# hackmad/pbrt-v3-rs

Measured on AMD Instinct MI355X. Metric: Mrays/s, higher is better.
Workload: dtype f32

## Files before the change

include/pbrt_hip.h:

```cpp
#ifndef PBRT_HIP_H
#define PBRT_HIP_H

#include <stddef.h>
#include <stdint.h>

#ifdef __cplusplus
extern "C" {
#endif

typedef struct PbrtHipScene PbrtHipScene;

enum {
    PBRT_HIP_OK = 0,
    PBRT_HIP_ERR_INVALID_ARG = -1,
    PBRT_HIP_ERR_STATE = -2,
    PBRT_HIP_ERR_DEVICE = -3,
    PBRT_HIP_ERR_NO_DEVICE = -4,
    PBRT_HIP_ERR_UNSUPPORTED = -5,
    PBRT_HIP_ERR_OOM = -6
};

typedef struct PbrtHipRay {
    float o[3];
    float t_max;
// ... 146 lines not shown
int pbrt_hip_occluded_batch_device(PbrtHipScene*, const void* d_rays, void* d_occluded, uint64_t n, float* kernel_ms);

int pbrt_hip_set_traversal_counting(PbrtHipScene*, int on);
int pbrt_hip_get_traversal_counts(PbrtHipScene*, uint64_t out[8]);

int pbrt_hip_render_path(PbrtHipScene*, int max_depth, float rr_threshold, int light_strategy,
                         const int pixel_bounds[4], int tile_size, int tile_part, int tile_parts,
                         float* out_xyz, float* out_weight, PbrtHipStats* out_stats);

int pbrt_hip_render_whitted(PbrtHipScene*, int max_depth, const int pixel_bounds[4], int tile_size, int tile_part, int tile_parts,
                            float* out_xyz, float* out_weight, PbrtHipStats* out_stats);

int pbrt_hip_set_sample_record_budget(PbrtHipScene*, uint64_t bytes);
int pbrt_hip_get_render_footprint(PbrtHipScene*, uint64_t out[8]);

int pbrt_hip_tile_buffer_floats(PbrtHipScene*, int tile_size, int tile_part, int tile_parts, uint64_t* out_floats);
int pbrt_hip_render_path_tiles_device(PbrtHipScene*, int max_depth, float rr_threshold, int light_strategy,
                                      const int pixel_bounds[4], int tile_size, int tile_part, int tile_parts,
                                      void* d_tile_buffer, PbrtHipStats* out_stats);
int pbrt_hip_merge_tiles_device(PbrtHipScene*, int tile_size, int tile_parts, const void* const* d_tile_buffers,
                                float* out_xyz, float* out_weight);

int pbrt_hip_film_to_rgb(const PbrtHipScene*, const float* xyz, const float* weight, float* out_rgb);

int pbrt_hip_generate_camera_rays(PbrtHipScene*, const int pixel_bounds[4], uint32_t sample_index,
                                  PbrtHipRay* out_rays, float* out_pfilm_xy);

int pbrt_hip_bsdf_probe_batch(PbrtHipScene*, uint32_t material, int op, int path, uint64_t n, const float* wo , const float* wi , const float* u ,
                              const uint32_t* flags , const float* frame , float* out );
int pbrt_hip_sampler_value_batch(PbrtHipScene*, uint64_t n, const int* xy , const uint32_t* sample , const uint32_t* dim , int use_lds, float* out );
#define PBRT_HIP_LIGHT_PROBE_STRIDE 28
int pbrt_hip_light_probe_batch(PbrtHipScene*, uint32_t light, int op, int variant, uint64_t n, const float* ref , const float* u , const float* wi ,
                               float* out );

#ifdef __cplusplus
}
#endif
#endif
```

pbrt-v3-rs_amd/csrc/probe.hip:

```cpp
#define PH_OUTLINE_MATH 1
#include "scene_host.h"
#include "pt_device.h"
#include "bsdf_general.h"
#include "wf_device.h"
#include "texture.h"
#include "sphere_light.h"
#include <cstring>

namespace ph {

struct ProbeFrame { float ns[3], ng[3], ss[3]; };
#define PH_PROBE_BLOCK 128

template <bool GEN>
__global__ __launch_bounds__(PH_PROBE_BLOCK) void bsdf_probe_kernel(DeviceScene sc, uint32_t material, int op, uint32_t n, const float* wo_in, const float* wi_in, const float* u_in,
                                                                   const uint32_t* flags_in, ProbeFrame fr, float* out) {
    const uint32_t i = blockIdx.x * blockDim.x + threadIdx.x;
    if (i >= n) return;
    SurfHit si;
    si.p = mk3(0.0f, 0.0f, 0.0f); si.p_error = si.p; si.wo = si.p; si.time = 0.0f; si.prim = 0u;
    si.ns = ld3(fr.ns); si.n = ld3(fr.ng); si.dpdu_s = ld3(fr.ss);
    const f3 wo = ld3(wo_in + 3 * (size_t)i), wi = ld3(wi_in + 3 * (size_t)i);
    const f2 u = mk2(u_in[2 * (size_t)i], u_in[2 * (size_t)i + 1]);
    const uint32_t flags = flags_in[i];
// ... 178 lines not shown
    const LightRec& l = s->lights[light];
    if (l.type == PH_L_AREA) {
        if (l.prim >= s->tri_mesh.size()) return set_err(s, PBRT_HIP_ERR_STATE, "light_probe_batch: the area light has no shape yet");
        if ((s->meshes[s->tri_mesh[l.prim]].flags & PH_MESH_QUADRIC) && variant != 2)
            return set_err(s, PBRT_HIP_ERR_UNSUPPORTED, "light_probe_batch: a spherical area light is sampled by the Whitted light loop alone (variant 2)");
    }
    if (variant == 1 && l.map_mip1) return set_err(s, PBRT_HIP_ERR_UNSUPPORTED, "light_probe_batch: variant 1 is the code of scenes without textures; this light holds a radiance, projection or goniometric map");
    if (n == 0) return PBRT_HIP_OK;
    PH_CHECK(s, hipSetDevice(s->device));
    int rc;
    if ((rc = upload_scene(s))) return rc;
    const size_t stride = PBRT_HIP_LIGHT_PROBE_STRIDE * sizeof(float);
    const size_t o_ref = 0, o_u = o_ref + up256(n * 40), o_wi = o_u + up256(n * 8), o_out = o_wi + up256(n * 12), total = o_out + up256(n * stride);
    Scratch sx;
    PH_CHECK(s, hipMalloc(&sx.p, total));
    char* d = static_cast<char*>(sx.p);
    PH_CHECK(s, hipMemcpyAsync(d + o_ref, ref, n * 40, hipMemcpyHostToDevice, s->stream));
    PH_CHECK(s, hipMemcpyAsync(d + o_u, u, n * 8, hipMemcpyHostToDevice, s->stream));
    PH_CHECK(s, hipMemcpyAsync(d + o_wi, wi, n * 12, hipMemcpyHostToDevice, s->stream));
    const dim3 grid((uint32_t)((n + PH_PROBE_BLOCK - 1) / PH_PROBE_BLOCK)), block(PH_PROBE_BLOCK);
    auto launch = [&](auto kernel) {
        hipLaunchKernelGGL(kernel, grid, block, 0, s->stream, s->ds, light, op, (uint32_t)n, (const float*)(d + o_ref), (const float*)(d + o_u), (const float*)(d + o_wi), (float*)(d + o_out));
    };
    if (variant == 0) launch(ph::light_probe_kernel<0>);
    else if (variant == 1) launch(ph::light_probe_kernel<1>);
    else launch(ph::light_probe_kernel<2>);
    PH_CHECK(s, hipGetLastError());
    PH_CHECK(s, hipMemcpyAsync(out, d + o_out, n * stride, hipMemcpyDeviceToHost, s->stream));
    PH_CHECK(s, hipStreamSynchronize(s->stream));
    return PBRT_HIP_OK;
    });
}

}
```

pbrt-v3-rs_amd/csrc/raysort.h:

```cpp
#pragma once
#include "traverse.h"

namespace ph {

#define PH_SORT_BINS 4096u
#define PH_SORT_KEYS (2u * PH_SORT_BINS)
#define PH_SORT_BLOCK 256

struct RaySortParams {
    const uint32_t* keys_cl; const uint32_t* keys_sh;
    const uint32_t* n_cl; const uint32_t* n_sh;
    uint32_t* order;
    uint32_t* bin_start;
    uint32_t* bin_cursor;
};
struct RaySortGrid {
    float lo[3], scale[3];
};

PH_DEV uint32_t part1by2(uint32_t v) {
    v &= 0xFu;
    v = (v | (v << 4)) & 0xC3u;
    v = (v | (v << 2)) & 0x249u;
    return v;
}

PH_DEV uint32_t ray_sort_key(const RaySortGrid& g, float ox, float oy, float oz) {
    const float fx = (ox - g.lo[0]) * g.scale[0], fy = (oy - g.lo[1]) * g.scale[1], fz = (oz - g.lo[2]) * g.scale[2];
    const uint32_t cx = (uint32_t)pmini(pmaxi((int)(fx * 16.0f), 0), 15);
    const uint32_t cy = (uint32_t)pmini(pmaxi((int)(fy * 16.0f), 0), 15);
    const uint32_t cz = (uint32_t)pmini(pmaxi((int)(fz * 16.0f), 0), 15);
    return part1by2(cx) | (part1by2(cy) << 1) | (part1by2(cz) << 2);
}
PH_DEV uint32_t raysort_key_at(const RaySortParams& p, uint32_t i, uint32_t n_cl) {
    return i < n_cl ? p.keys_cl[i] : PH_SORT_BINS + p.keys_sh[i - n_cl];
}

PH_DEV void raysort_slice(const RaySortParams& p, uint32_t n, uint32_t& lo, uint32_t& hi) {
    const uint32_t per = (((n + gridDim.x - 1u) / gridDim.x) + PH_SORT_BLOCK - 1u) & ~(uint32_t)(PH_SORT_BLOCK - 1u);
    lo = blockIdx.x * per; hi = lo + per < n ? lo + per : n;
    if (lo > n) lo = n;
}

__global__ __launch_bounds__(PH_SORT_BLOCK) void raysort_hist_kernel(RaySortParams p) {
    __shared__ uint32_t h[PH_SORT_KEYS];
    const uint32_t n_cl = *p.n_cl, n = n_cl + *p.n_sh;
    uint32_t lo, hi;
    raysort_slice(p, n, lo, hi);
    if (lo >= hi) return;
    for (uint32_t k = threadIdx.x; k < PH_SORT_KEYS; k += PH_SORT_BLOCK) h[k] = 0u;
    __syncthreads();
    for (uint32_t i = lo + threadIdx.x; i < hi; i += PH_SORT_BLOCK) atomicAdd(&h[raysort_key_at(p, i, n_cl)], 1u);
    __syncthreads();
    for (uint32_t k = threadIdx.x; k < PH_SORT_KEYS; k += PH_SORT_BLOCK)
        if (h[k]) atomicAdd(&p.bin_start[k], h[k]);
}

__global__ __launch_bounds__(1024) void raysort_scan_kernel(RaySortParams p) {
    __shared__ uint32_t part[1024];
    constexpr uint32_t PER = PH_SORT_KEYS / 1024u;
    uint32_t v[PER], sum = 0u;
    for (uint32_t k = 0; k < PER; k++) { v[k] = p.bin_start[threadIdx.x * PER + k]; sum += v[k]; }
    part[threadIdx.x] = sum;
    __syncthreads();
    for (uint32_t o = 1; o < 1024u; o <<= 1) {
        const uint32_t add = threadIdx.x >= o ? part[threadIdx.x - o] : 0u;
        __syncthreads();
        part[threadIdx.x] += add;
        __syncthreads();
    }
    uint32_t run = part[threadIdx.x] - sum;
    for (uint32_t k = 0; k < PER; k++) { p.bin_start[threadIdx.x * PER + k] = run; p.bin_cursor[threadIdx.x * PER + k] = 0u; run += v[k]; }
}

__global__ __launch_bounds__(PH_SORT_BLOCK) void raysort_scatter_kernel(RaySortParams p) {
    __shared__ uint32_t h[PH_SORT_KEYS];
    __shared__ uint32_t base[PH_SORT_KEYS];
    const uint32_t n_cl = *p.n_cl, n = n_cl + *p.n_sh;
    uint32_t lo, hi;
    raysort_slice(p, n, lo, hi);
    if (lo >= hi) return;
    for (uint32_t k = threadIdx.x; k < PH_SORT_KEYS; k += PH_SORT_BLOCK) h[k] = 0u;
    __syncthreads();
    for (uint32_t i = lo + threadIdx.x; i < hi; i += PH_SORT_BLOCK) atomicAdd(&h[raysort_key_at(p, i, n_cl)], 1u);
    __syncthreads();
    for (uint32_t k = threadIdx.x; k < PH_SORT_KEYS; k += PH_SORT_BLOCK) {
        const uint32_t c = h[k];
        base[k] = c ? p.bin_start[k] + atomicAdd(&p.bin_cursor[k], c) : 0u;
        h[k] = 0u;
    }
    __syncthreads();
    for (uint32_t i = lo + threadIdx.x; i < hi; i += PH_SORT_BLOCK) {
        const uint32_t key = raysort_key_at(p, i, n_cl);
        p.order[base[key] + atomicAdd(&h[key], 1u)] = i;
    }
}

}
```

pbrt-v3-rs_amd/csrc/scene_host.h:

```cpp
#pragma once
#include "../../include/pbrt_hip.h"
#include "band_plan.h"
#include "bvh_build.h"
#include "guard.h"
#include "scene_types.h"
#include <hip/hip_runtime.h>
namespace ph { struct TravParams; }
#include <string>
#include <vector>

struct DevBuf {
    void* p = nullptr;
    size_t bytes = 0;
};

struct SceneHostState {
    std::vector<float> P, N, S, UV;
    bool any_n = false, any_s = false, any_uv = false;
    std::vector<uint32_t> idx, tri_mesh, tri_flags;
    std::vector<MeshRec> meshes;
    std::vector<QuadricRec> quadrics;
    std::vector<float> quadric_bounds;
    std::vector<uint32_t> prim_quadric;
    std::vector<MaterialRec> materials;
    std::vector<LobeRec> lobes;
    struct TextureHost { std::vector<TexOp> prog; int stack_need = 1; };
    std::vector<TextureHost> textures;
    std::vector<MipRec> mipmaps;
    std::vector<Texel> texels;
    struct MaterialParams { int lobe[4] = {-1, -1, -1, -1}; int field[4] = {0, 0, 0, 0}; int lobe2[4] = {-1, -1, -1, -1}; int field2[4] = {0, 0, 0, 0}; bool has_pre = false; float pre[3] = {1, 1, 1}; int rough_lobe = -1, rough_lobe2 = -1; bool rough_remap = false;
                            int made_as = 0;   float raw_k[4][3] = {{0, 0, 0}, {0, 0, 0}, {0, 0, 0}, {0, 0, 0}}; float raw_eta = 1.5f, raw_ur = 0, raw_vr = 0;
                            bool raw_remap = false, rebuilt = false; int mix_n1 = 0; };
    std::vector<MaterialParams> material_params;
    bool alpha_textures = false;
    bool alpha_lean = false;
    bool bump_materials = false;
    bool textured_materials = false;
// ... 33 lines not shown
    MultiDevice* multi = nullptr;

    DeviceScene ds{};
    std::vector<void*> owned;
    void* tree_dev_nodes = nullptr; void* tree_dev_tris = nullptr; size_t tree_dev_n_tris = 0;
    bool uploaded = false;
    int light_strategy_uploaded = -1;
    DevBuf d_ld_func, d_ld_cdf;

    DevBuf d_counter, d_spill, d_error, d_rays_tmp, d_out_tmp;
    uint32_t trav_blocks = 0;
    bool count_traversal = false;
    DevBuf d_counts;
    hipEvent_t ev0 = nullptr, ev1 = nullptr;

    struct Wavefront* wf = nullptr;
    struct WhittedWorkspace* wh = nullptr;

    uint64_t record_budget = 0;
    uint64_t footprint[8] = {0, 0, 0, 0, 0, 0, 0, 0};
};

namespace phost {
int set_err(PbrtHipScene* s, int code, const std::string& msg);
int hip_fail(PbrtHipScene* s, hipError_t e, const char* what);
int ensure_buf(PbrtHipScene* s, DevBuf& b, size_t bytes);
int upload_scene(PbrtHipScene* s);
void projection_light_setup(float fov_deg, float aspect, float out_proj[16], float out_screen[4], float* out_cos_total_width);
void hmip_lookup_triangle(const PbrtHipScene* s, const MipRec& m, float u, float v, float width, float out[3]);
int upload_light_distribution(PbrtHipScene* s, int light_strategy);
int launch_traverse(PbrtHipScene* s, bool anyhit, const void* d_rays, void* d_out, uint32_t n, float* kernel_ms);
void launch_traverse_kernel(PbrtHipScene* s, int mode, uint32_t blocks, const ph::TravParams& p);
int ensure_traversal_workspace(PbrtHipScene* s);
void free_wavefront(PbrtHipScene* s);
int build_hlbvh_device(const BuildInput& in, int max_prims_in_node, hipStream_t stream, BuildOutput& out, std::string& err, const ForestSpec* forest = nullptr,
                       std::vector<ForestTreeOut>* trees_out = nullptr);
int build_sah_device(const BuildInput& in, int max_prims_in_node, hipStream_t stream, BuildOutput& out, std::string& err, void** keep_nodes = nullptr, void** keep_tris = nullptr,
                     const ForestSpec* forest = nullptr, std::vector<ForestTreeOut>* trees_out = nullptr);
void free_tree_dev(PbrtHipScene* s);
int uber_rebuild_for_opacity(PbrtHipScene* s, uint32_t material);
int glass_rebuild_for_roughness(PbrtHipScene* s, uint32_t material);
int translucent_rebuild_rt(PbrtHipScene* s, uint32_t material);
#define PH_MAX_TILE_PARTS 64
int check_render_args(PbrtHipScene* s, int max_depth, int light_strategy, const int* pixel_bounds, int tile_size, int part, int parts);
size_t tile_buffer_floats_for(const PbrtHipScene* s, int tile_size, int part, int parts);
int render_tiles(PbrtHipScene* s, int max_depth, float rr_threshold, int light_strategy, const int pixel_bounds[4], int tile_size, int part, int parts, void* d_tile_buffer,
                 PbrtHipStats* out_stats);
int merge_tiles(PbrtHipScene* s, int tile_size, int parts, const void* const* d_bufs, float* out_xyz, float* out_weight);
DevBuf& tile_buffer_of(PbrtHipScene* s);
int merge_own_tiles(PbrtHipScene* s, int tile_size, int tile_part, int tile_parts, float* out_xyz, float* out_weight);
struct SampleRecords { uint32_t n_px; const int2* px_xy; float4* rec_L; float* rec_py; uint8_t* px_rounded; SampleBand band; uint32_t band_px; std::vector<SampleBand> bands; };
int samples_begin(PbrtHipScene* s, int tile_size, int part, int parts, SampleRecords* out);
int samples_plan_bands(PbrtHipScene* s, SampleRecords* out, size_t chunk_held, size_t chunk_per_path);
int samples_alloc(PbrtHipScene* s, SampleRecords* out);
int samples_band(PbrtHipScene* s, const SampleRecords& r, size_t band, SampleRecords* out);
int samples_to_tiles(PbrtHipScene* s, const SampleRecords& r, void* d_tile_buffer);
size_t path_chunk_bytes_per_path(bool general_materials, bool textured_materials);
void free_whitted(PbrtHipScene* s);
size_t whitted_chunk_bytes_per_sample(uint32_t n_frames);
int spatial_voxels_touched(PbrtHipScene* s, std::vector<uint8_t>& touched, uint64_t* count);
int render_path_multi(PbrtHipScene* s, int max_depth, float rr_threshold, int light_strategy, const int pixel_bounds[4], int tile_size, int tile_part, int tile_parts,
                      float* out_xyz, float* out_weight, PbrtHipStats* out_stats);
void free_multi(PbrtHipScene* s);
}

#define PH_CHECK(s, call)                                              \
// ... 5 lines not shown
```

pbrt-v3-rs_amd/csrc/wavefront.hip:

```cpp
#define PH_OUTLINE_MATH 1
#include "host_math.h"
#include "pt_device.h"
#include "scene_host.h"
#include "spatial.h"
#include "bsdf_general.h"
#include "texture.h"
#include "raysort.h"
#include "phase_clock.h"
#include "matsort.h"
#include "wf_device.h"
#include "chunk_plan.h"
#include <algorithm>
#include <cstdlib>

namespace ph {

enum : uint32_t { F_EXT = 1u, F_PSH = 2u, F_PMIS = 4u, F_SPEC = 8u, F_NODIFF = 16u };

struct IterCounters {
    uint32_t n_cl, n_sh, n_live, head_cl, head_sh, pad[3];
};
struct DevStats { unsigned long long camera_rays, paths_total, paths_zero; };

struct TileInfo {
// ... 666 lines not shown
    int tiles_key[12] = {0}; bool tiles_valid = false;
    DevBuf d_tiles, d_px, d_rays_cl[2], d_hits, d_rays_sh, d_occ, d_live[2], d_ctr, d_stats, d_cam, d_tex_out;
    DevBuf d_sL, d_sbeta, d_sA, d_sf2, d_sbold, d_sidx, d_sprev, d_recL, d_recpy, d_rounded, d_tilebuf, d_xyz, d_w;
    DevBuf d_vox_slot, d_sp_pool, d_sp_list, d_sp_ctr, d_sp_halton;
    DevBuf d_order, d_sort_bins, d_heads, d_keys_cl, d_keys_sh;
    DevBuf d_morder, d_mkeys, d_mbins;
    size_t n_vox = 0;
    std::vector<hipEvent_t> events;
    phost::ChunkTable chunk_table(bool textured, bool mat_queues) {
        const size_t ray = sizeof(ph::RayIn), hit = sizeof(ph::HitOut);
        return {{&d_rays_cl[0], 2 * ray}, {&d_rays_cl[1], 2 * ray}, {&d_hits, 2 * hit}, {&d_rays_sh, ray}, {&d_occ, 1}, {&d_live[0], 4}, {&d_live[1], 4},
                {&d_sL, 2 * 16}, {&d_sbeta, 2 * 16}, {&d_sA, 2 * 16}, {&d_sf2, 2 * 16}, {&d_sbold, 2 * 16}, {&d_sidx, 2 * 16}, {&d_sprev, 2 * 4},
                {&d_order, 3 * 4}, {&d_keys_cl, 2 * 4}, {&d_keys_sh, 4}, {&d_tex_out, textured ? sizeof(TexOut) : 0, textured}, {&d_morder, 4, mat_queues}, {&d_mkeys, 2, mat_queues}};
    }
    std::vector<DevBuf*> all_bufs() {
        std::vector<DevBuf*> v{&d_tiles, &d_px, &d_ctr, &d_stats, &d_cam, &d_recL, &d_recpy, &d_rounded, &d_tilebuf, &d_xyz, &d_w,
                               &d_vox_slot, &d_sp_pool, &d_sp_list, &d_sp_ctr, &d_sp_halton, &d_sort_bins, &d_heads, &d_mbins};
        for (const phost::ChunkBuf& c : chunk_table(false, false)) v.push_back(c.buf);
        return v;
    }
};

namespace phost {

void free_wavefront(PbrtHipScene* s) {
    Wavefront* w = s->wf;
    if (!w) return;
    for (DevBuf* b : w->all_bufs()) release_buf(*b);
    for (hipEvent_t e : w->events) (void)hipEventDestroy(e);
    delete w;
    s->wf = nullptr;
}

size_t path_chunk_bytes_per_path(bool general, bool textured) { Wavefront w; return chunk_bytes_per_path(w.chunk_table(textured, general || textured)); }
static int sat_i(float v) { if (v != v) return 0; if (v >= 2147483648.0f) return 2147483647; if (v <= -2147483648.0f) return (int)0x80000000; return (int)v; }

struct TileGrid { int sb[4]; int ntx, nty; uint32_t slot_w, slot_h; };
static TileGrid tile_grid(const FilmRec& f, int tile_size) {
    TileGrid g;
    g.sb[0] = sat_i(std::floor((float)f.crop[0] + 0.5f - f.radius[0])); g.sb[1] = sat_i(std::floor((float)f.crop[1] + 0.5f - f.radius[1]));
    g.sb[2] = sat_i(std::ceil((float)f.crop[2] - 0.5f + f.radius[0])); g.sb[3] = sat_i(std::ceil((float)f.crop[3] - 0.5f + f.radius[1]));
    g.ntx = std::max((g.sb[2] - g.sb[0] + tile_size - 1) / tile_size, 0); g.nty = std::max((g.sb[3] - g.sb[1] + tile_size - 1) / tile_size, 0);
    const int e_lo_x = sat_i(std::floor(0.5f + f.radius[0])), e_hi_x = sat_i(std::floor(f.radius[0] - 0.5f)) + 1;
    const int e_lo_y = sat_i(std::floor(0.5f + f.radius[1])), e_hi_y = sat_i(std::floor(f.radius[1] - 0.5f)) + 1;
    g.slot_w = (uint32_t)std::max(tile_size + e_lo_x + e_hi_x, 1); g.slot_h = (uint32_t)std::max(tile_size + e_lo_y + e_hi_y, 1);
    return g;
}

static int setup_tiles(PbrtHipScene* s, int tile_size, int part, int parts) {
    if (!s->wf) s->wf = new Wavefront();
    Wavefront& w = *s->wf;
    const FilmRec& f = s->film;
    const TileGrid g = tile_grid(f, tile_size);
    int key[12] = {f.crop[0], f.crop[1], f.crop[2], f.crop[3], 0, 0, tile_size, part, parts, g.ntx, g.nty, 1};
    std::memcpy(&key[4], &f.radius[0], 4); std::memcpy(&key[5], &f.radius[1], 4);
    if (w.tiles_valid && std::memcmp(key, w.tiles_key, sizeof key) == 0) return PBRT_HIP_OK;
    w.tiles_valid = false;
    const int* sb = g.sb; const int ntx = g.ntx, nty = g.nty;
    w.tiles.clear(); w.px_xy.clear();
    std::memcpy(w.sb, sb, sizeof(w.sb)); w.ntx = ntx; w.nty = nty; w.tile_size = tile_size; w.part = part; w.parts = parts;
    w.slot_w = g.slot_w; w.slot_h = g.slot_h;
    for (int t = part; t < ntx * nty; t += parts) {
        ph::TileInfo ti{};
        const int tx = t % ntx, ty = t / ntx;
        ti.tb[0] = sb[0] + tx * tile_size; ti.tb[2] = std::min(ti.tb[0] + tile_size, sb[2]);
        ti.tb[1] = sb[1] + ty * tile_size; ti.tb[3] = std::min(ti.tb[1] + tile_size, sb[3]);
// ... 95 lines not shown
                        int parts, void* d_tile_buffer, PbrtHipStats* out_stats) {
    int rc;
    PH_CHECK(s, hipSetDevice(s->device));
    if ((rc = upload_scene(s))) return rc;
    const bool spatial = light_strategy == 2 && s->lights.size() > 1;
    if ((rc = upload_light_distribution(s, light_strategy == 2 ? 0 : light_strategy))) return rc;
    if (out_stats) std::memset(out_stats, 0, sizeof(*out_stats));
    SampleRecords rec{};
    if ((rc = samples_begin(s, tile_size, part, parts, &rec))) return rc;
    Wavefront& w = *s->wf;
    const uint32_t spp = s->sampler.spp;
    if (rec.n_px == 0) { PH_CHECK(s, hipMemsetAsync(d_tile_buffer, 0, tile_buffer_floats_for(s, tile_size, part, parts) * 4, s->stream)); PH_CHECK(s, hipStreamSynchronize(s->stream)); return PBRT_HIP_OK; }

    static const ChunkPolicy kChunks{128u << 20, 1u << 20, 0x7FFF0000ull, "render"};
    const bool mat_queues = s->general_materials || s->textured_materials;
    const ChunkTable chunk = w.chunk_table(s->textured_materials, mat_queues);
    if ((rc = samples_plan_bands(s, &rec, chunk_bytes_held(chunk), chunk_bytes_per_path(chunk)))) return rc;
    const uint32_t n_px = rec.band_px;
    const size_t rec_need = (size_t)n_px * spp * 20, rec_have = w.d_recL.bytes + w.d_recpy.bytes;
    uint32_t chunk_spp = plan_chunk_spp_now(kChunks, chunk, rec_need > rec_have ? rec_need - rec_have : 0, n_px, spp);
    const int n_iter = max_depth + 1;
    const int kMaxNullSkips = 1024;
    const int n_iter_cap = s->has_none_material ? n_iter + kMaxNullSkips : n_iter;
    const bool has_quadrics = !s->quadrics.empty();
    if ((rc = ensure_buf(s, w.d_ctr, (size_t)(n_iter_cap + 2) * sizeof(ph::IterCounters)))) return rc;
    if ((rc = ensure_buf(s, w.d_stats, 64 + 6 * PHC_N * 8))) return rc;
    if ((rc = samples_alloc(s, &rec))) return rc;
    if ((rc = chunk_alloc_or_halve(s, kChunks, chunk, n_px, chunk_spp))) return rc;
    const size_t B = (size_t)n_px * chunk_spp;
    chunk_note_footprint(s, B, chunk);

    if ((rc = ensure_traversal_workspace(s))) return rc;
    const uint32_t n_heads = 8, head_chunk = 49152, sort_blocks = 1024;
    ph::RaySortParams sortp{};
    ph::RaySortGrid sort_grid{};
    if ((rc = ensure_buf(s, w.d_sort_bins, 2 * PH_SORT_KEYS * 4))) return rc;
    sortp.order = (uint32_t*)w.d_order.p; sortp.bin_start = (uint32_t*)w.d_sort_bins.p; sortp.bin_cursor = sortp.bin_start + PH_SORT_KEYS;
    sortp.keys_cl = (const uint32_t*)w.d_keys_cl.p; sortp.keys_sh = (const uint32_t*)w.d_keys_sh.p;
    for (int k = 0; k < 3; k++) {
        const float ext = s->bvh.root_hi[k] - s->bvh.root_lo[k];
        sort_grid.lo[k] = s->bvh.root_lo[k]; sort_grid.scale[k] = ext > 0.0f ? 1.0f / ext : 0.0f;
    }
    if ((rc = ensure_buf(s, w.d_heads, (size_t)(n_iter_cap + 2) * n_heads * 64))) return rc;
    ph::MatSortParams msp{};
    if (mat_queues) {
        if ((rc = ensure_buf(s, w.d_mbins, (size_t)(2 * PH_MS_BINS + 1) * 4))) return rc;
        msp.max_depth = max_depth; msp.mat_key = s->ds.mat_key; msp.key_emit = s->ds.ms_key_emit; msp.key_idle = s->ds.ms_key_idle;
        msp.tris = s->ds.tris; msp.meshes = s->ds.meshes; msp.hits = (const ph::HitOut*)w.d_hits.p;
        msp.keys = (uint16_t*)w.d_mkeys.p; msp.order = (uint32_t*)w.d_morder.p;
        msp.bin_start = (uint32_t*)w.d_mbins.p; msp.bin_cursor = msp.bin_start + PH_MS_BINS + 1;
    }

    ph::WfParams wp{};
    wp.cam = s->cam; wp.sp = s->sampler;
    wp.textured = s->textured_materials ? 1u : 0u; wp.cam_dev = nullptr;
    wp.any_rt = 0u;
    for (const MaterialRec& mr : s->materials) if (mr.rt_mode) wp.any_rt = 1u;
    if (s->textured_materials) {
        if ((rc = ensure_buf(s, w.d_cam, sizeof(CameraRec)))) return rc;
        PH_CHECK(s, hipMemcpyAsync(w.d_cam.p, &s->cam, sizeof(CameraRec), hipMemcpyHostToDevice, s->stream));
        wp.cam_dev = (const CameraRec*)w.d_cam.p;
    }
    for (int i = 0; i < 4; i++) wp.pixel_bounds[i] = pixel_bounds[i];
    wp.max_depth = max_depth; wp.rr_threshold = rr_threshold;
    wp.rays_cl[0] = (ph::RayIn*)w.d_rays_cl[0].p; wp.rays_cl[1] = (ph::RayIn*)w.d_rays_cl[1].p;
    wp.hits_cl = (ph::HitOut*)w.d_hits.p; wp.rays_sh = (ph::RayIn*)w.d_rays_sh.p; wp.occ = (uint8_t*)w.d_occ.p;
    wp.live[0] = (uint32_t*)w.d_live[0].p; wp.live[1] = (uint32_t*)w.d_live[1].p;
    wp.ctr = (ph::IterCounters*)w.d_ctr.p; wp.stats = (ph::DevStats*)w.d_stats.p;
    for (int k = 0; k < 2; k++) {
        wp.s_L[k] = (float4*)w.d_sL.p + (size_t)k * B; wp.s_beta[k] = (float4*)w.d_sbeta.p + (size_t)k * B; wp.s_A[k] = (float4*)w.d_sA.p + (size_t)k * B;
        wp.s_f2[k] = (float4*)w.d_sf2.p + (size_t)k * B; wp.s_bold[k] = (float4*)w.d_sbold.p + (size_t)k * B; wp.s_idx[k] = (uint4*)w.d_sidx.p + (size_t)k * B;
// ... 27 lines not shown
    uint64_t regular = 0, shadow = 0;
    std::vector<ph::IterCounters> hctr((size_t)n_iter_cap + 2);
    const uint32_t shade_blocks = (uint32_t)std::min<size_t>((B + 255) / 256, 256 * 16);
    wp.tex_out = nullptr;
    if (s->textured_materials) wp.tex_out = (TexOut*)w.d_tex_out.p;

    for (size_t band = 0; band < rec.bands.size(); band++) {
        SampleRecords br{};
        if ((rc = samples_band(s, rec, band, &br))) return rc;
        wp.n_px = br.n_px; wp.px_xy = br.px_xy; wp.rec_L = br.rec_L; wp.rec_py = br.rec_py; wp.px_rounded = br.px_rounded;
        for (uint32_t s0 = 0; s0 < spp; s0 += chunk_spp) {
            const uint32_t cs = std::min(chunk_spp, spp - s0);
            wp.chunk_spp = cs; wp.s0 = s0; wp.B = br.n_px * cs; wp.identity_slots = identity ? 1u : 0u;
            PH_CHECK(s, hipMemsetAsync(w.d_ctr.p, 0, (size_t)(n_iter_cap + 2) * sizeof(ph::IterCounters), s->stream));
            PH_CHECK(s, hipMemsetAsync(w.d_heads.p, 0, (size_t)(n_iter_cap + 2) * n_heads * 64, s->stream));
            if (identity) hipLaunchKernelGGL(ph::preset_counters_kernel, dim3(1), dim3(1), 0, s->stream, wp.ctr, wp.stats, wp.B);
            if ((rc = timed(2, [&]() { hipLaunchKernelGGL(ph::raygen_kernel, dim3((wp.B + 255) / 256), dim3(256), 0, s->stream, s->ds, wp); }))) return rc;
            int iters_run = 0;
            for (int it = 0; it < n_iter_cap; it++) {
                ph::IterCounters* c = (ph::IterCounters*)w.d_ctr.p + it;
                if (it >= n_iter) {
                    uint32_t live = 0;
                    PH_CHECK(s, hipMemcpyAsync(&live, &c->n_live, 4, hipMemcpyDeviceToHost, s->stream));
                    PH_CHECK(s, hipStreamSynchronize(s->stream));
                    if (live == 0) break;
                    if (it == n_iter_cap - 1) return set_err(s, PBRT_HIP_ERR_UNSUPPORTED, "render: a path crossed more than 1024 'none' surfaces");
                }
                iters_run = it + 1;
                ph::TravParams tp{};
                tp.rays = wp.rays_cl[it & 1]; tp.out = wp.hits_cl; tp.n = 0; tp.n_ptr = &c->n_cl; tp.counter = &c->head_cl;
                tp.heads = (uint32_t*)w.d_heads.p + (size_t)it * n_heads * 16; tp.n_heads = n_heads; tp.head_chunk = head_chunk;
                if (it > 0) {
                    tp.rays2 = wp.rays_sh; tp.out2 = wp.occ; tp.n2_ptr = &c->n_sh;
                    sortp.n_cl = &c->n_cl; sortp.n_sh = &c->n_sh;
                    if ((rc = timed(3, [&]() {
                            (void)hipMemsetAsync(sortp.bin_start, 0, PH_SORT_KEYS * 4, s->stream);
                            hipLaunchKernelGGL(ph::raysort_hist_kernel, dim3(sort_blocks), dim3(PH_SORT_BLOCK), 0, s->stream, sortp);
                            hipLaunchKernelGGL(ph::raysort_scan_kernel, dim3(1), dim3(1024), 0, s->stream, sortp);
                            hipLaunchKernelGGL(ph::raysort_scatter_kernel, dim3(sort_blocks), dim3(PH_SORT_BLOCK), 0, s->stream, sortp);
                        }))) return rc;
                    tp.order = sortp.order;
                    if ((rc = timed(0, [&]() { launch_traverse_kernel(s, 2, s->trav_blocks, tp); }))) return rc;
                } else if ((rc = timed(0, [&]() { launch_traverse_kernel(s, 0, s->trav_blocks, tp); }))) return rc;
                if (mat_queues) {
                    msp.s_idx = wp.s_idx[it & 1]; msp.n_live = &c->n_live;
                    if ((rc = timed(2, [&]() {
                            (void)hipMemsetAsync(msp.bin_start, 0, (PH_MS_BINS + 1) * 4, s->stream);
                            hipLaunchKernelGGL(ph::matsort_hist_kernel, dim3(sort_blocks), dim3(PH_MS_BLOCK), 0, s->stream, msp);
                            hipLaunchKernelGGL(ph::matsort_scan_kernel, dim3(1), dim3(PH_MS_BINS), 0, s->stream, msp);
                            hipLaunchKernelGGL(ph::matsort_scatter_kernel, dim3(sort_blocks), dim3(PH_MS_BLOCK), 0, s->stream, msp);
                        }))) return rc;
                }
                if (s->textured_materials) {
                    if ((rc = timed(2, [&]() {
                            const dim3 g(shade_blocks), b(PH_TEX_LDS_THREADS);
                            if (it == 0) {
                                if (has_quadrics) hipLaunchKernelGGL((ph::texture_kernel<false, true, 2, true>), g, b, 0, s->stream, s->ds, wp, it);
                                else if (s->simple_textures) hipLaunchKernelGGL((ph::texture_kernel<true, true, 3>), g, b, 0, s->stream, s->ds, wp, it);
                                else hipLaunchKernelGGL((ph::texture_kernel<false, true, 2>), g, b, 0, s->stream, s->ds, wp, it);
                            } else {
                                if (has_quadrics) hipLaunchKernelGGL((ph::texture_kernel<false, false, 3, true>), g, b, 0, s->stream, s->ds, wp, it);
                                else if (s->simple_textures) hipLaunchKernelGGL((ph::texture_kernel<true, false, 4>), g, b, 0, s->stream, s->ds, wp, it);
                                else hipLaunchKernelGGL((ph::texture_kernel<false, false, 3>), g, b, 0, s->stream, s->ds, wp, it);
                            }
                        }))) return rc;
                }
                if (spatial && (it < max_depth || s->has_none_material)) {
                    if ((rc = timed(2, [&]() {
                            if (has_quadrics) hipLaunchKernelGGL(ph::spatial_mark_kernel<true>, dim3(shade_blocks), dim3(256), 0, s->stream, s->ds, wp, it);
                            else hipLaunchKernelGGL(ph::spatial_mark_kernel<false>, dim3(shade_blocks), dim3(256), 0, s->stream, s->ds, wp, it);
                            hipLaunchKernelGGL(ph::spatial_compute_kernel, dim3(1024), dim3(PH_SPATIAL_BLOCK), 0, s->stream, s->ds, wp.spatial);
                        }))) return rc;
                }
                if ((rc = timed(2, [&]() {
// ... 281 lines not shown
```

pbrt-v3-rs_amd/pbrt_hip/__init__.py:

```python
from __future__ import annotations

import ctypes as C
import os
from dataclasses import dataclass

import numpy as np

_HERE = os.path.dirname(os.path.abspath(__file__))
LIB_PATH = os.environ.get("PBRT_HIP_LIB") or os.path.join(os.path.dirname(_HERE), "libpbrt_hip.so")

OK = 0
ERR_INVALID_ARG, ERR_STATE, ERR_DEVICE, ERR_NO_DEVICE, ERR_UNSUPPORTED, ERR_OOM = -1, -2, -3, -4, -5, -6

RAY_DTYPE = np.dtype([("o", "<f4", 3), ("t_max", "<f4"), ("d", "<f4", 3), ("time", "<f4")])
HIT_DTYPE = np.dtype([("t", "<f4"), ("prim", "<u4"), ("b0", "<f4"), ("b1", "<f4"), ("b2", "<f4"), ("pad", "<u4", 3)])
assert RAY_DTYPE.itemsize == 32 and HIT_DTYPE.itemsize == 32


class Stats(C.Structure):
    _fields_ = [
        ("camera_rays", C.c_uint64), ("regular_rays", C.c_uint64), ("shadow_rays", C.c_uint64),
        ("paths_zero_radiance", C.c_uint64), ("paths_total", C.c_uint64),
        ("render_seconds", C.c_double), ("extend_seconds", C.c_double), ("shadow_seconds", C.c_double),
        ("shade_seconds", C.c_double), ("extend_launches", C.c_uint64), ("shadow_launches", C.c_uint64),
# ... 93 lines not shown
            "add_texture_checkerboard": (C.c_int, [vp, C.c_uint32, C.c_uint32, C.c_float, C.c_float, C.c_float, C.c_float, C.c_int, u32p]),
            "add_texture_uv": (C.c_int, [vp, C.c_float, C.c_float, C.c_float, C.c_float, u32p]),
            "add_texture_bilerp": (C.c_int, [vp, fp, fp, fp, fp, C.c_float, C.c_float, C.c_float, C.c_float, u32p]),
            "add_texture_dots": (C.c_int, [vp, C.c_uint32, C.c_uint32, C.c_float, C.c_float, C.c_float, C.c_float, u32p]),
            "add_light_infinite_map": (C.c_int, [vp, fp, C.c_int, C.c_int, fp, fp, fp]),
            "add_texture_fbm": (C.c_int, [vp, fp, C.c_float, C.c_int, u32p]),
            "add_texture_wrinkled": (C.c_int, [vp, fp, C.c_float, C.c_int, u32p]),
            "add_texture_windy": (C.c_int, [vp, fp, u32p]),
            "add_texture_marble": (C.c_int, [vp, fp, C.c_float, C.c_int, C.c_float, C.c_float, u32p]),
            "add_texture_checkerboard3d": (C.c_int, [vp, C.c_uint32, C.c_uint32, fp, u32p]),
            "set_texture_mapping": (C.c_int, [vp, C.c_uint32, C.c_int, fp]),
            "add_material_matte_tex": (C.c_int, [vp, C.c_uint32, C.c_float, u32p]),
            "set_material_texture": (C.c_int, [vp, C.c_uint32, C.c_int, C.c_uint32]),
            "set_material_bump": (C.c_int, [vp, C.c_uint32, C.c_uint32]),
            "set_material_float_texture": (C.c_int, [vp, C.c_uint32, C.c_int, C.c_uint32]),
            "set_last_mesh_alpha_textures": (C.c_int, [vp, C.c_uint32, C.c_uint32]),
            "texture_eval_batch": (C.c_int, [vp, C.c_uint32, C.c_uint64, fp, fp]),
            "texture_eval_batch_nodiff": (C.c_int, [vp, C.c_uint32, C.c_uint64, fp, fp]),
            "mipmap_levels": (C.c_int, [vp, C.c_uint32, ip, ip]),
            "mipmap_level_texels": (C.c_int, [vp, C.c_uint32, C.c_int, fp]),
            "set_traversal_counting": (C.c_int, [vp, C.c_int]),
            "get_traversal_counts": (C.c_int, [vp, C.POINTER(C.c_uint64)]),
            "accel_stats": (C.c_int, [vp, C.POINTER(C.c_uint64)]),
            "accel_copy": (C.c_int, [vp, vp, C.c_uint64, vp, C.c_uint64]),
            "build_accel_device": (C.c_int, [vp, C.c_int, C.c_int]),
            "scene_create_multi": (vp, [ip, C.c_int]),
            "scene_devices": (C.c_int, [vp, ip, C.c_int]),
            "selftest_rccl_gather": (C.c_int, [vp, C.c_uint32, C.POINTER(C.c_uint64)]),
            "set_sample_record_budget": (C.c_int, [vp, C.c_uint64]),
            "get_render_footprint": (C.c_int, [vp, C.POINTER(C.c_uint64)]),
            "bsdf_probe_batch": (C.c_int, [vp, C.c_uint32, C.c_int, C.c_int, C.c_uint64, fp, fp, fp, u32p, fp, fp]),
            "sampler_value_batch": (C.c_int, [vp, C.c_uint64, ip, u32p, u32p, C.c_int, fp]),
            "light_probe_batch": (C.c_int, [vp, C.c_uint32, C.c_int, C.c_int, C.c_uint64, fp, fp, fp, fp]),
        }
        for name, (res, args) in self._optional.items():
            if hasattr(self.lib, prefix + name):
                fn = f(name)
                fn.restype, fn.argtypes = res, args

    def fn(self, name):
        return getattr(self.lib, self.prefix + name)

    def has(self, name):
        return hasattr(self.lib, self.prefix + name)


_default = None


def default_binding() -> Binding:
    global _default
    if _default is None:
        _default = Binding(LIB_PATH, "pbrt_hip_")
    return _default


class Host:

    def __init__(self, binding: Binding | None = None):
        b = binding or default_binding()
        self.lib = b.lib
        fp = C.POINTER(C.c_float)
        L = self.lib
        L.pbrt_hip_host_look_at.restype = C.c_int
        L.pbrt_hip_host_gen_random_tris.argtypes = [C.c_uint64, C.c_uint64, fp, C.POINTER(C.c_uint32)]
        L.pbrt_hip_host_rotate.argtypes = [C.c_float, fp, fp, fp]
# ... 741 lines not shown
```

Measured before the change: 2326.

## Restructure ray sort: per-block bin offsets from histogram, vectorized key walks

The histogram pass now stores each block's starting offset per bin, which it gets from the global atomic. The scatter pass therefore no longer recounts its slice and no longer needs the cursor atomics. Keys are read as aligned uint4 vectors, several loads are kept in flight per thread, and duplicate bins within a vector are combined into one LDS atomic. Each slice now has a minimum size (floor of 16384 keys), so small queues use fewer blocks. In exchange, a per-block share table of sort_blocks×8192 words is added, and scatter order within a bin is no longer deterministic. A host-side probe entry point is also added for testing the sort.

```diff
diff --git a/include/pbrt_hip.h b/include/pbrt_hip.h
--- a/include/pbrt_hip.h
+++ b/include/pbrt_hip.h
@@ -202,6 +202,7 @@
 #define PBRT_HIP_LIGHT_PROBE_STRIDE 28
 int pbrt_hip_light_probe_batch(PbrtHipScene*, uint32_t light, int op, int variant, uint64_t n, const float* ref , const float* u , const float* wi ,
                                float* out );
+int pbrt_hip_raysort_probe(PbrtHipScene*, uint32_t n_cl, uint32_t n_sh, const uint32_t* keys_cl, const uint32_t* keys_sh, uint32_t sort_blocks, uint32_t* order_out );
 
 #ifdef __cplusplus
 }
diff --git a/pbrt-v3-rs_amd/csrc/probe.hip b/pbrt-v3-rs_amd/csrc/probe.hip
--- a/pbrt-v3-rs_amd/csrc/probe.hip
+++ b/pbrt-v3-rs_amd/csrc/probe.hip
@@ -234,4 +234,31 @@
     });
 }
 
-}
+int pbrt_hip_raysort_probe(PbrtHipScene* s, uint32_t n_cl, uint32_t n_sh, const uint32_t* keys_cl, const uint32_t* keys_sh, uint32_t sort_blocks, uint32_t* order_out) {
+    return ph_guard(s, "pbrt_hip_raysort_probe", [&]() -> int {
+    if (!s || (n_cl && !keys_cl) || (n_sh && !keys_sh) || ((n_cl || n_sh) && !order_out)) return set_err(s, PBRT_HIP_ERR_INVALID_ARG, "raysort_probe: null argument");
+    if (sort_blocks == 0 || sort_blocks > 65536u) return set_err(s, PBRT_HIP_ERR_INVALID_ARG, "raysort_probe: sort_blocks must be 1 .. 65536");
+    const uint64_t n = (uint64_t)n_cl + n_sh;
+    if (n >= 0x7FFF0000ull) return set_err(s, PBRT_HIP_ERR_INVALID_ARG, "raysort_probe: more rays than a round's queues hold");
+    for (uint32_t i = 0; i < n_cl; i++) if (keys_cl[i] >= PH_SORT_BINS) return set_err(s, PBRT_HIP_ERR_INVALID_ARG, "raysort_probe: a key is not below 4096");
+    for (uint32_t i = 0; i < n_sh; i++) if (keys_sh[i] >= PH_SORT_BINS) return set_err(s, PBRT_HIP_ERR_INVALID_ARG, "raysort_probe: a key is not below 4096");
+    PH_CHECK(s, hipSetDevice(s->device));
+    const size_t o_cl = 0, o_sh = o_cl + up256((size_t)n_cl * 4), o_n = o_sh + up256((size_t)n_sh * 4), o_order = o_n + 256, o_ws = o_order + up256(n * 4),
+                 total = o_ws + up256(raysort_workspace_bytes(sort_blocks));
+    Scratch sx;
+    PH_CHECK(s, hipMalloc(&sx.p, total));
+    char* d = static_cast<char*>(sx.p);
+    const uint32_t counts[2] = {n_cl, n_sh};
+    if (n_cl) PH_CHECK(s, hipMemcpyAsync(d + o_cl, keys_cl, (size_t)n_cl * 4, hipMemcpyHostToDevice, s->stream));
+    if (n_sh) PH_CHECK(s, hipMemcpyAsync(d + o_sh, keys_sh, (size_t)n_sh * 4, hipMemcpyHostToDevice, s->stream));
+    PH_CHECK(s, hipMemcpyAsync(d + o_n, counts, 8, hipMemcpyHostToDevice, s->stream));
+    launch_raysort(s, (const uint32_t*)(d + o_cl), (const uint32_t*)(d + o_sh), (const uint32_t*)(d + o_n), (const uint32_t*)(d + o_n) + 1, (uint32_t*)(d + o_order), (uint32_t*)(d + o_ws),
+                   sort_blocks);
+    PH_CHECK(s, hipGetLastError());
+    if (n) PH_CHECK(s, hipMemcpyAsync(order_out, d + o_order, n * 4, hipMemcpyDeviceToHost, s->stream));
+    PH_CHECK(s, hipStreamSynchronize(s->stream));
+    return PBRT_HIP_OK;
+    });
+}
+
+}
diff --git a/pbrt-v3-rs_amd/csrc/raysort.h b/pbrt-v3-rs_amd/csrc/raysort.h
--- a/pbrt-v3-rs_amd/csrc/raysort.h
+++ b/pbrt-v3-rs_amd/csrc/raysort.h
@@ -1,18 +1,17 @@
 #pragma once
+#include "raysort_plan.h"
 #include "traverse.h"
 
 namespace ph {
 
-#define PH_SORT_BINS 4096u
-#define PH_SORT_KEYS (2u * PH_SORT_BINS)
-#define PH_SORT_BLOCK 256
+#define PH_SORT_DEPTH 4
 
 struct RaySortParams {
     const uint32_t* keys_cl; const uint32_t* keys_sh;
     const uint32_t* n_cl; const uint32_t* n_sh;
     uint32_t* order;
     uint32_t* bin_start;
-    uint32_t* bin_cursor;
+    uint32_t* block_share;
 };
 struct RaySortGrid {
     float lo[3], scale[3];
@@ -32,28 +31,59 @@
     const uint32_t cz = (uint32_t)pmini(pmaxi((int)(fz * 16.0f), 0), 15);
     return part1by2(cx) | (part1by2(cy) << 1) | (part1by2(cz) << 2);
 }
-PH_DEV uint32_t raysort_key_at(const RaySortParams& p, uint32_t i, uint32_t n_cl) {
-    return i < n_cl ? p.keys_cl[i] : PH_SORT_BINS + p.keys_sh[i - n_cl];
+template <class FV, class F1>
+PH_DEV void raysort_walk_run(const uint32_t* keys, const RaySortRun& r, uint32_t key_add, uint32_t pos_add, FV&& fv, F1&& f1) {
+    if (r.head + threadIdx.x < r.body) f1(keys[r.head + threadIdx.x] + key_add, r.head + threadIdx.x + pos_add);
+    const uint4* body = reinterpret_cast<const uint4*>(keys + r.body);
+    const uint32_t n_vec = (r.tail - r.body) >> 2;
+    uint32_t j = threadIdx.x;
+    for (; j + (PH_SORT_DEPTH - 1) * PH_SORT_BLOCK < n_vec; j += PH_SORT_DEPTH * PH_SORT_BLOCK) {
+        uint4 v[PH_SORT_DEPTH];
+#pragma unroll
+        for (uint32_t d = 0; d < PH_SORT_DEPTH; d++) v[d] = body[j + d * PH_SORT_BLOCK];
+        __builtin_amdgcn_sched_barrier(0);
+#pragma unroll
+        for (uint32_t d = 0; d < PH_SORT_DEPTH; d++) { v[d].x += key_add; v[d].y += key_add; v[d].z += key_add; v[d].w += key_add; }
+        fv(v, r.body + 4u * j + pos_add);
+    }
+    for (; j < n_vec; j += PH_SORT_BLOCK) {
+        const uint4 v = body[j];
+        const uint32_t i = r.body + 4u * j + pos_add;
+        f1(v.x + key_add, i); f1(v.y + key_add, i + 1u); f1(v.z + key_add, i + 2u); f1(v.w + key_add, i + 3u);
+    }
+    if (r.tail + threadIdx.x < r.end) f1(keys[r.tail + threadIdx.x] + key_add, r.tail + threadIdx.x + pos_add);
 }
-
-PH_DEV void raysort_slice(const RaySortParams& p, uint32_t n, uint32_t& lo, uint32_t& hi) {
-    const uint32_t per = (((n + gridDim.x - 1u) / gridDim.x) + PH_SORT_BLOCK - 1u) & ~(uint32_t)(PH_SORT_BLOCK - 1u);
-    lo = blockIdx.x * per; hi = lo + per < n ? lo + per : n;
-    if (lo > n) lo = n;
+template <class FV, class F1>
+PH_DEV void raysort_walk_slice(const RaySortParams& p, const RaySortSlice& s, uint32_t n_cl, FV&& fv, F1&& f1) {
+    raysort_walk_run(p.keys_cl, s.cl, 0u, 0u, fv, f1);
+    raysort_walk_run(p.keys_sh, s.sh, PH_SORT_BINS, n_cl, fv, f1);
 }
+PH_DEV RaySortSlice raysort_slice(const RaySortParams& p, uint32_t n_cl, uint32_t n_sh) {
+    return raysort_plan(n_cl, n_sh, gridDim.x, PH_SORT_BLOCK, PH_SORT_FLOOR, blockIdx.x, (uint32_t)((uintptr_t)p.keys_cl >> 2) & 3u, (uint32_t)((uintptr_t)p.keys_sh >> 2) & 3u);
+}
+PH_DEV uint32_t raysort_bin(uint32_t key) { return key & (PH_SORT_KEYS - 1u); }
 
 __global__ __launch_bounds__(PH_SORT_BLOCK) void raysort_hist_kernel(RaySortParams p) {
     __shared__ uint32_t h[PH_SORT_KEYS];
-    const uint32_t n_cl = *p.n_cl, n = n_cl + *p.n_sh;
-    uint32_t lo, hi;
-    raysort_slice(p, n, lo, hi);
-    if (lo >= hi) return;
+    const uint32_t n_cl = *p.n_cl, n_sh = *p.n_sh;
+    const RaySortSlice s = raysort_slice(p, n_cl, n_sh);
+    if (s.lo >= s.hi) return;
     for (uint32_t k = threadIdx.x; k < PH_SORT_KEYS; k += PH_SORT_BLOCK) h[k] = 0u;
     __syncthreads();
-    for (uint32_t i = lo + threadIdx.x; i < hi; i += PH_SORT_BLOCK) atomicAdd(&h[raysort_key_at(p, i, n_cl)], 1u);
+    raysort_walk_slice(p, s, n_cl,
+        [&](const uint4 (&v)[PH_SORT_DEPTH], uint32_t) {
+#pragma unroll
+            for (uint32_t d = 0; d < PH_SORT_DEPTH; d++) {
+                atomicAdd(&h[raysort_bin(v[d].x)], 1u); atomicAdd(&h[raysort_bin(v[d].y)], 1u); atomicAdd(&h[raysort_bin(v[d].z)], 1u); atomicAdd(&h[raysort_bin(v[d].w)], 1u);
+            }
+        },
+        [&](uint32_t key, uint32_t) { atomicAdd(&h[raysort_bin(key)], 1u); });
     __syncthreads();
-    for (uint32_t k = threadIdx.x; k < PH_SORT_KEYS; k += PH_SORT_BLOCK)
-        if (h[k]) atomicAdd(&p.bin_start[k], h[k]);
+    uint32_t* share = p.block_share + (size_t)blockIdx.x * PH_SORT_KEYS;
+    for (uint32_t k = threadIdx.x; k < PH_SORT_KEYS; k += PH_SORT_BLOCK) {
+        const uint32_t c = h[k];
+        share[k] = c ? atomicAdd(&p.bin_start[k], c) : 0u;
+    }
 }
 
 __global__ __launch_bounds__(1024) void raysort_scan_kernel(RaySortParams p) {
@@ -70,30 +100,41 @@
         __syncthreads();
     }
     uint32_t run = part[threadIdx.x] - sum;
-    for (uint32_t k = 0; k < PER; k++) { p.bin_start[threadIdx.x * PER + k] = run; p.bin_cursor[threadIdx.x * PER + k] = 0u; run += v[k]; }
+    for (uint32_t k = 0; k < PER; k++) { p.bin_start[threadIdx.x * PER + k] = run; run += v[k]; }
 }
 
 __global__ __launch_bounds__(PH_SORT_BLOCK) void raysort_scatter_kernel(RaySortParams p) {
-    __shared__ uint32_t h[PH_SORT_KEYS];
     __shared__ uint32_t base[PH_SORT_KEYS];
-    const uint32_t n_cl = *p.n_cl, n = n_cl + *p.n_sh;
-    uint32_t lo, hi;
-    raysort_slice(p, n, lo, hi);
-    if (lo >= hi) return;
-    for (uint32_t k = threadIdx.x; k < PH_SORT_KEYS; k += PH_SORT_BLOCK) h[k] = 0u;
+    const uint32_t n_cl = *p.n_cl, n_sh = *p.n_sh;
+    const RaySortSlice s = raysort_slice(p, n_cl, n_sh);
+    if (s.lo >= s.hi) return;
+    const uint32_t* share = p.block_share + (size_t)blockIdx.x * PH_SORT_KEYS;
+    for (uint32_t k = threadIdx.x; k < PH_SORT_KEYS; k += PH_SORT_BLOCK) base[k] = p.bin_start[k] + share[k];
     __syncthreads();
-    for (uint32_t i = lo + threadIdx.x; i < hi; i += PH_SORT_BLOCK) atomicAdd(&h[raysort_key_at(p, i, n_cl)], 1u);
-    __syncthreads();
-    for (uint32_t k = threadIdx.x; k < PH_SORT_KEYS; k += PH_SORT_BLOCK) {
-        const uint32_t c = h[k];
-        base[k] = c ? p.bin_start[k] + atomicAdd(&p.bin_cursor[k], c) : 0u;
-        h[k] = 0u;
-    }
-    __syncthreads();
-    for (uint32_t i = lo + threadIdx.x; i < hi; i += PH_SORT_BLOCK) {
-        const uint32_t key = raysort_key_at(p, i, n_cl);
-        p.order[base[key] + atomicAdd(&h[key], 1u)] = i;
-    }
+    raysort_walk_slice(p, s, n_cl,
+        [&](const uint4 (&v)[PH_SORT_DEPTH], uint32_t i0) {
+            uint4 at[PH_SORT_DEPTH];
+#pragma unroll
+            for (uint32_t d = 0; d < PH_SORT_DEPTH; d++) {
+                const uint32_t x = raysort_bin(v[d].x), y = raysort_bin(v[d].y), z = raysort_bin(v[d].z), w = raysort_bin(v[d].w);
+                const uint32_t yx = y == x, zx = z == x, wx = w == x, zy = z == y, wy = w == y, wz = w == z;
+                at[d].x = atomicAdd(&base[x], 1u + yx + zx + wx);
+                at[d].y = yx ? 0u : atomicAdd(&base[y], 1u + zy + wy);
+                at[d].z = (zx | zy) ? 0u : atomicAdd(&base[z], 1u + wz);
+                at[d].w = (wx | wy | wz) ? 0u : atomicAdd(&base[w], 1u);
+            }
+#pragma unroll
+            for (uint32_t d = 0; d < PH_SORT_DEPTH; d++) {
+                const uint32_t x = raysort_bin(v[d].x), y = raysort_bin(v[d].y), z = raysort_bin(v[d].z), w = raysort_bin(v[d].w);
+                const uint32_t yx = y == x, zx = z == x, wx = w == x, zy = z == y, wy = w == y, wz = w == z;
+                const uint32_t rx = at[d].x, ry = yx ? rx + 1u : at[d].y;
+                const uint32_t rz = zx ? rx + 1u + yx : zy ? ry + 1u : at[d].z;
+                const uint32_t rw = wx ? rx + 1u + yx + zx : wy ? ry + 1u + zy : wz ? rz + 1u : at[d].w;
+                const uint32_t i = i0 + 4u * d * PH_SORT_BLOCK;
+                p.order[rx] = i; p.order[ry] = i + 1u; p.order[rz] = i + 2u; p.order[rw] = i + 3u;
+            }
+        },
+        [&](uint32_t key, uint32_t i) { p.order[atomicAdd(&base[raysort_bin(key)], 1u)] = i; });
 }
 
 }
diff --git a/pbrt-v3-rs_amd/csrc/raysort_plan.h b/pbrt-v3-rs_amd/csrc/raysort_plan.h
--- /dev/null
+++ b/pbrt-v3-rs_amd/csrc/raysort_plan.h
@@ -0,0 +1,48 @@
+#pragma once
+#include <cstdint>
+
+namespace ph {
+
+#define PH_SORT_BINS 4096u
+#define PH_SORT_KEYS (2u * PH_SORT_BINS)
+#define PH_SORT_BLOCK 256
+#define PH_SORT_FLOOR 16384u
+
+#if defined(__HIPCC__)
+#define PH_PLAN_HD __host__ __device__ inline
+#else
+#define PH_PLAN_HD inline
+#endif
+
+struct RaySortRun { uint32_t head, body, tail, end; };
+struct RaySortSlice { uint32_t lo, hi; RaySortRun cl, sh; };
+
+PH_PLAN_HD uint32_t raysort_slice_keys(uint32_t n, uint32_t grid, uint32_t block, uint32_t floor) {
+    const uint32_t each = (n + grid - 1u) / grid;
+    const uint32_t per = (each + block - 1u) / block * block;
+    return per > floor ? per : floor;
+}
+
+PH_PLAN_HD RaySortRun raysort_run(uint32_t a, uint32_t e, uint32_t mis) {
+    RaySortRun r;
+    r.head = a; r.end = e;
+    const uint32_t to_boundary = (4u - ((a + mis) & 3u)) & 3u;
+    r.body = e - a < to_boundary ? e : a + to_boundary;
+    r.tail = r.body + ((e - r.body) & ~3u);
+    return r;
+}
+
+PH_PLAN_HD RaySortSlice raysort_plan(uint32_t n_cl, uint32_t n_sh, uint32_t grid, uint32_t block, uint32_t floor, uint32_t b, uint32_t mis_cl, uint32_t mis_sh) {
+    const uint32_t n = n_cl + n_sh;
+    const uint64_t per = raysort_slice_keys(n, grid, block, floor);
+    const uint64_t lo64 = (uint64_t)b * per, hi64 = lo64 + per;
+    RaySortSlice s;
+    s.lo = lo64 < n ? (uint32_t)lo64 : n;
+    s.hi = hi64 < n ? (uint32_t)hi64 : n;
+    const uint32_t cl_a = s.lo < n_cl ? s.lo : n_cl, cl_e = s.hi < n_cl ? s.hi : n_cl;
+    s.cl = raysort_run(cl_a, cl_e, mis_cl);
+    s.sh = raysort_run(s.lo - cl_a, s.hi - cl_e, mis_sh);
+    return s;
+}
+
+}
diff --git a/pbrt-v3-rs_amd/csrc/scene_host.h b/pbrt-v3-rs_amd/csrc/scene_host.h
--- a/pbrt-v3-rs_amd/csrc/scene_host.h
+++ b/pbrt-v3-rs_amd/csrc/scene_host.h
@@ -3,6 +3,7 @@
 #include "band_plan.h"
 #include "bvh_build.h"
 #include "guard.h"
+#include "raysort_plan.h"
 #include "scene_types.h"
 #include <hip/hip_runtime.h>
 namespace ph { struct TravParams; }
@@ -102,6 +103,9 @@
 int launch_traverse(PbrtHipScene* s, bool anyhit, const void* d_rays, void* d_out, uint32_t n, float* kernel_ms);
 void launch_traverse_kernel(PbrtHipScene* s, int mode, uint32_t blocks, const ph::TravParams& p);
 int ensure_traversal_workspace(PbrtHipScene* s);
+inline size_t raysort_workspace_bytes(uint32_t sort_blocks) { return ((size_t)sort_blocks + 1) * PH_SORT_KEYS * 4; }
+void launch_raysort(PbrtHipScene* s, const uint32_t* keys_cl, const uint32_t* keys_sh, const uint32_t* n_cl, const uint32_t* n_sh, uint32_t* order, uint32_t* workspace,
+                    uint32_t sort_blocks);
 void free_wavefront(PbrtHipScene* s);
 int build_hlbvh_device(const BuildInput& in, int max_prims_in_node, hipStream_t stream, BuildOutput& out, std::string& err, const ForestSpec* forest = nullptr,
                        std::vector<ForestTreeOut>* trees_out = nullptr);
diff --git a/pbrt-v3-rs_amd/csrc/wavefront.hip b/pbrt-v3-rs_amd/csrc/wavefront.hip
--- a/pbrt-v3-rs_amd/csrc/wavefront.hip
+++ b/pbrt-v3-rs_amd/csrc/wavefront.hip
@@ -722,6 +722,16 @@
     s->wf = nullptr;
 }
 
+void launch_raysort(PbrtHipScene* s, const uint32_t* keys_cl, const uint32_t* keys_sh, const uint32_t* n_cl, const uint32_t* n_sh, uint32_t* order, uint32_t* workspace,
+                    uint32_t sort_blocks) {
+    ph::RaySortParams p{};
+    p.keys_cl = keys_cl; p.keys_sh = keys_sh; p.n_cl = n_cl; p.n_sh = n_sh; p.order = order; p.bin_start = workspace; p.block_share = workspace + PH_SORT_KEYS;
+    (void)hipMemsetAsync(p.bin_start, 0, PH_SORT_KEYS * 4, s->stream);
+    hipLaunchKernelGGL(ph::raysort_hist_kernel, dim3(sort_blocks), dim3(PH_SORT_BLOCK), 0, s->stream, p);
+    hipLaunchKernelGGL(ph::raysort_scan_kernel, dim3(1), dim3(1024), 0, s->stream, p);
+    hipLaunchKernelGGL(ph::raysort_scatter_kernel, dim3(sort_blocks), dim3(PH_SORT_BLOCK), 0, s->stream, p);
+}
+
 size_t path_chunk_bytes_per_path(bool general, bool textured) { Wavefront w; return chunk_bytes_per_path(w.chunk_table(textured, general || textured)); }
 static int sat_i(float v) { if (v != v) return 0; if (v >= 2147483648.0f) return 2147483647; if (v <= -2147483648.0f) return (int)0x80000000; return (int)v; }
 
@@ -883,11 +893,8 @@
 
     if ((rc = ensure_traversal_workspace(s))) return rc;
     const uint32_t n_heads = 8, head_chunk = 49152, sort_blocks = 1024;
-    ph::RaySortParams sortp{};
     ph::RaySortGrid sort_grid{};
-    if ((rc = ensure_buf(s, w.d_sort_bins, 2 * PH_SORT_KEYS * 4))) return rc;
-    sortp.order = (uint32_t*)w.d_order.p; sortp.bin_start = (uint32_t*)w.d_sort_bins.p; sortp.bin_cursor = sortp.bin_start + PH_SORT_KEYS;
-    sortp.keys_cl = (const uint32_t*)w.d_keys_cl.p; sortp.keys_sh = (const uint32_t*)w.d_keys_sh.p;
+    if ((rc = ensure_buf(s, w.d_sort_bins, raysort_workspace_bytes(sort_blocks)))) return rc;
     for (int k = 0; k < 3; k++) {
         const float ext = s->bvh.root_hi[k] - s->bvh.root_lo[k];
         sort_grid.lo[k] = s->bvh.root_lo[k]; sort_grid.scale[k] = ext > 0.0f ? 1.0f / ext : 0.0f;
@@ -981,14 +988,9 @@
                 tp.heads = (uint32_t*)w.d_heads.p + (size_t)it * n_heads * 16; tp.n_heads = n_heads; tp.head_chunk = head_chunk;
                 if (it > 0) {
                     tp.rays2 = wp.rays_sh; tp.out2 = wp.occ; tp.n2_ptr = &c->n_sh;
-                    sortp.n_cl = &c->n_cl; sortp.n_sh = &c->n_sh;
-                    if ((rc = timed(3, [&]() {
-                            (void)hipMemsetAsync(sortp.bin_start, 0, PH_SORT_KEYS * 4, s->stream);
-                            hipLaunchKernelGGL(ph::raysort_hist_kernel, dim3(sort_blocks), dim3(PH_SORT_BLOCK), 0, s->stream, sortp);
-                            hipLaunchKernelGGL(ph::raysort_scan_kernel, dim3(1), dim3(1024), 0, s->stream, sortp);
-                            hipLaunchKernelGGL(ph::raysort_scatter_kernel, dim3(sort_blocks), dim3(PH_SORT_BLOCK), 0, s->stream, sortp);
-                        }))) return rc;
-                    tp.order = sortp.order;
+                    uint32_t* const order = (uint32_t*)w.d_order.p;
+                    if ((rc = timed(3, [&]() { launch_raysort(s, wp.keys_cl, wp.keys_sh, &c->n_cl, &c->n_sh, order, (uint32_t*)w.d_sort_bins.p, sort_blocks); }))) return rc;
+                    tp.order = order;
                     if ((rc = timed(0, [&]() { launch_traverse_kernel(s, 2, s->trav_blocks, tp); }))) return rc;
                 } else if ((rc = timed(0, [&]() { launch_traverse_kernel(s, 0, s->trav_blocks, tp); }))) return rc;
                 if (mat_queues) {
diff --git a/pbrt-v3-rs_amd/pbrt_hip/__init__.py b/pbrt-v3-rs_amd/pbrt_hip/__init__.py
--- a/pbrt-v3-rs_amd/pbrt_hip/__init__.py
+++ b/pbrt-v3-rs_amd/pbrt_hip/__init__.py
@@ -149,6 +149,7 @@
             "bsdf_probe_batch": (C.c_int, [vp, C.c_uint32, C.c_int, C.c_int, C.c_uint64, fp, fp, fp, u32p, fp, fp]),
             "sampler_value_batch": (C.c_int, [vp, C.c_uint64, ip, u32p, u32p, C.c_int, fp]),
             "light_probe_batch": (C.c_int, [vp, C.c_uint32, C.c_int, C.c_int, C.c_uint64, fp, fp, fp, fp]),
+            "raysort_probe": (C.c_int, [vp, C.c_uint32, C.c_uint32, u32p, u32p, C.c_uint32, u32p]),
         }
         for name, (res, args) in self._optional.items():
             if hasattr(self.lib, prefix + name):
```

Measured after the change: 2356, median of 6. +1.3%, better.
